# strukturag/libheif

Measured on NVIDIA H100. Metric: megapixels/sec HEIC-grid decode->RGB, higher is better.
Workload: dtype u8

## Files before the change

### libheif_b200/csrc/b200_hevc_entropy.cu

```cuda
#include <cstdint>
#include <cstdlib>
namespace b200 { namespace syn {
__shared__ uint32_t s_kLps4[64];
__shared__ uint8_t s_kTransLps[64];
__shared__ uint8_t s_kNextState[256];
__shared__ unsigned long long s_kState[128];
__shared__ uint8_t s_kInitI[135];
__shared__ uint8_t s_kSigMap4[16];
__shared__ uint8_t s_kScanPos[3][16];
__shared__ uint8_t s_kScanInv[3][16];
__shared__ uint8_t s_kSbInv[4][3][64];
__shared__ uint8_t s_kSigCtx4[3][16];
__shared__ uint8_t s_kSigCtxN[3][4][16];
__shared__ uint8_t s_kChromaTab[4];
__shared__ uint8_t s_kScanX[4][3][64];
__shared__ uint8_t s_kScanY[4][3][64];
} }
#ifdef __CUDA_ARCH__
#define B200_T(name) s_##name
#endif
#include "b200_hevc.h"
static_assert(b200::syn::CTX_COUNT == 135, "s_kInitI above is sized for 135 context variables");

namespace b200 {

#ifndef B200_ENTROPY_WARPS
#define B200_ENTROPY_WARPS 4
#endif
constexpr int EWARPS = B200_ENTROPY_WARPS;

__device__ __forceinline__ unsigned e_ld_acquire(const unsigned* p) {
  unsigned v; asm volatile("ld.relaxed.gpu.global.u32 %0, [%1];" : "=r"(v) : "l"(p) : "memory"); return v;
}
__device__ __forceinline__ void e_st_release(unsigned* p, unsigned v) {
  asm volatile("st.release.gpu.global.u32 [%0], %1;" ::"l"(p), "r"(v) : "memory");
}

struct DevSync {
  unsigned* progress;
  unsigned* sub_done;
  unsigned* error_flag;
  unsigned* queue; unsigned* qtail; unsigned* deps;
  uint32_t dense_tu, dense_coef, dense_tu_cap, dense_coef_cap;
  uint64_t end_bit_position;
  __device__ static void spin_until(const unsigned* p, unsigned need, unsigned* error_flag) {
    if (e_ld_acquire(p) >= need) return;
    unsigned ns = 200, spins = 0;
    for (;;) {
      __nanosleep(ns); if (ns < 8000) ns <<= 1;
      if (e_ld_acquire(p) >= need) return;
      if ((++spins & 63u) != 0) continue;
      if (e_ld_acquire(error_flag)) return;
      if (spins > (1u << 23)) { atomicExch(error_flag, 3u); return; }
    }
  }
  __device__ void wait_row(int row, int need) { spin_until(progress + row, (unsigned)need, error_flag); }
  __device__ void publish_row(int row, int done) { e_st_release(progress + row, (unsigned)done); }
  __device__ void wait_substream(int idx) { spin_until(sub_done + idx, 1u, error_flag); }
  __device__ void finish_substream(int idx, int err) {
    e_st_release(sub_done + idx, 1u);
    if (err) atomicExch(error_flag, (unsigned)err);
  }
  __device__ void notify(int target) {
    if (target < 0) return;
    __threadfence();
    if (atomicSub(deps + target, 1u) == 1u) { const unsigned s = atomicAdd(qtail, 1u); e_st_release(queue + s, (unsigned)target + 1u); }
  }
};

#ifndef B200_ENTROPY_MIN_BLOCKS
#define B200_ENTROPY_MIN_BLOCKS 1
#endif
#ifndef B200_ENTROPY_MAX_BLOCKS_PER_SM
#define B200_ENTROPY_MAX_BLOCKS_PER_SM 0
#endif
template <class Cfg> constexpr int entropy_min_blocks() { return B200_ENTROPY_MIN_BLOCKS; }
template <> constexpr int entropy_min_blocks<syn::CfgCommon>() { return B200_ENTROPY_MIN_BLOCKS > 5 ? B200_ENTROPY_MIN_BLOCKS : 5; }
template <class Cfg>
__global__ void __launch_bounds__(EWARPS * 32, entropy_min_blocks<Cfg>()) hevc_entropy_kernel(const EntropyBatch b) {
  __shared__ __align__(8) syn::U2 s_ctx[EWARPS][syn::CTX_COUNT];
  __shared__ syn::DecoderT<Cfg> s_dec[EWARPS];
  __shared__ DevSync s_sync[EWARPS];
  for (int i = threadIdx.x; i < 64; i += blockDim.x) { syn::s_kLps4[i] = syn::d_kLps4[i]; syn::s_kTransLps[i] = syn::d_kTransLps[i]; }
  for (int i = threadIdx.x; i < syn::CTX_COUNT; i += blockDim.x) syn::s_kInitI[i] = syn::d_kInitI[i];
  for (int i = threadIdx.x; i < 256; i += blockDim.x) syn::s_kNextState[i] = syn::d_kNextState[i];
  for (int i = threadIdx.x; i < 128; i += blockDim.x) syn::s_kState[i] = syn::d_kState[i];
  for (int i = threadIdx.x; i < 16; i += blockDim.x) syn::s_kSigMap4[i] = syn::d_kSigMap4[i];
  for (int i = threadIdx.x; i < 48; i += blockDim.x) { (&syn::s_kScanPos[0][0])[i] = (&syn::d_kScanPos[0][0])[i]; (&syn::s_kScanInv[0][0])[i] = (&syn::d_kScanInv[0][0])[i]; (&syn::s_kSigCtx4[0][0])[i] = (&syn::d_kSigCtx4[0][0])[i]; }
  for (int i = threadIdx.x; i < 192; i += blockDim.x) (&syn::s_kSigCtxN[0][0][0])[i] = (&syn::d_kSigCtxN[0][0][0])[i];
  for (int i = threadIdx.x; i < 768; i += blockDim.x) (&syn::s_kSbInv[0][0][0])[i] = (&syn::d_kSbInv[0][0][0])[i];
  for (int i = threadIdx.x; i < 4; i += blockDim.x) syn::s_kChromaTab[i] = syn::d_kChromaTab[i];
  for (int i = threadIdx.x; i < 4 * 3 * 64; i += blockDim.x) { (&syn::s_kScanX[0][0][0])[i] = (&syn::d_kScanX[0][0][0])[i]; (&syn::s_kScanY[0][0][0])[i] = (&syn::d_kScanY[0][0][0])[i]; }
  __syncthreads();
  if ((threadIdx.x & 31) != 0) return;
  const int slot_w = threadIdx.x >> 5;
  const syn::CtxPtr ctx = (syn::CtxPtr)__cvta_generic_to_shared(s_ctx[slot_w]);
  for (;;) {
    const unsigned slot = atomicAdd(b.qhead, 1u);
    if (slot >= (unsigned)b.nsubs) break;
    unsigned item = e_ld_acquire(b.queue + slot);
    if (!item) {
      unsigned ns = 500, spins = 0;
      for (;;) {
        __nanosleep(ns); if (ns < 16000) ns <<= 1;
        if ((item = e_ld_acquire(b.queue + slot)) != 0u) break;
        if ((++spins & 31u) != 0) continue;
        if (e_ld_acquire(b.error_flag)) return;
        if (spins > (1u << 22)) { atomicExch(b.error_flag, 3u); return; }
      }
    }
    const syn::Substream& gs = b.subs[item - 1u];
    const EntropyPic& ep = b.pics[gs.pic];
    DevSync& sync = s_sync[slot_w];
    sync.progress = b.progress + ep.progress_base; sync.sub_done = b.sub_done + ep.sub_base; sync.error_flag = b.error_flag;
    sync.queue = b.queue; sync.qtail = b.qtail; sync.deps = b.deps;
    sync.dense_tu = sync.dense_coef = sync.dense_tu_cap = sync.dense_coef_cap = 0; sync.end_bit_position = 0;
    syn::run_substream<Cfg>(s_dec[slot_w], ep.sp, ep.pb, b.subs + ep.sub_base, (int)(item - 1u - ep.sub_base), ctx, sync);
  }
}

__global__ void entropy_stats_kernel(const EntropyBatch b, unsigned long long* out2) {
  const int pi = blockIdx.y;
  const EntropyPic& ep = b.pics[pi];
  const int nctb = ep.sp.wctb * ep.sp.hctb;
  unsigned long long tus = 0, coefs = 0;
  for (int a = blockIdx.x * blockDim.x + threadIdx.x; a < nctb; a += gridDim.x * blockDim.x) {
    const CtuInfo ci = ep.pb.ctus[a];
    tus += ci.tu_count;
    for (unsigned k = 0; k < ci.tu_count; k++) { const TuCmd t = ep.pb.tus[ci.tu_start + k]; coefs += (t.w3 & 0x7ff) + ((t.w3 >> 11) & 0x3ff) + ((t.w3 >> 21) & 0x3ff); }
  }
  atomicAdd(out2, tus); atomicAdd(out2 + 1, coefs);
}

__global__ void entropy_gate_kernel(const unsigned* qhead, unsigned need, const unsigned* error_flag) {
// ... 50 lines not shown
```

### libheif_b200/csrc/b200_hevc_syntax.h

```cpp
#pragma once
#include <cstdint>
#include <cstring>
#include "b200_hevc_types.h"

#if defined(__CUDA_ARCH__) && !defined(B200_SYNTAX_HOST_ONLY)
#define B200_SYN_DEVICE 1
#endif
#if defined(__CUDACC__) && !defined(B200_SYNTAX_HOST_ONLY)
#define B200_HDN __host__ __device__ __noinline__
#define B200_NOUNROLL _Pragma("unroll 1")
#define B200_HD __host__ __device__
#define B200_HDI __host__ __device__ __forceinline__
#define B200_TABLE(type, name, dims, ...) static const type h_##name dims = __VA_ARGS__; static __device__ const type d_##name dims = __VA_ARGS__;
#else
#define B200_HDN
#define B200_NOUNROLL
#define B200_HD
#define B200_HDI inline
#define B200_TABLE(type, name, dims, ...) static const type h_##name dims = __VA_ARGS__;
#endif
#if defined(B200_SYN_DEVICE) && !defined(B200_T)
#define B200_T(name) d_##name
#endif
#ifdef B200_SYN_DEVICE
// ... 23 lines not shown
struct U2 { uint32_t x, y; };
typedef U2* CtxPtr;
typedef const uint8_t* TabPtr;
inline U2 ctx_ld(CtxPtr p) { return *p; }
inline void ctx_st(CtxPtr p, U2 v) { *p = v; }
inline CtxPtr ctx_at(CtxPtr base, int i) { return base + i; }
inline uint32_t tab_ld8(TabPtr p, int i) { return p[i]; }
inline uint32_t tab_ld32(TabPtr p, int i) { uint32_t v; memcpy(&v, p + 4 * (size_t)i, 4); return v; }
inline U2 tab_ld64(TabPtr p, int i) { uint64_t v; memcpy(&v, p + 8 * (size_t)i, 8); return U2{(uint32_t)v, (uint32_t)(v >> 32)}; }
#define B200_TADDR(name) (reinterpret_cast<::b200::syn::TabPtr>(&B200_T(name)))
#endif

enum { CTX_SAO_MERGE = 0, CTX_SAO_TYPE = 1, CTX_SPLIT_CU = 2, CTX_PART_MODE = 5, CTX_PREV_INTRA = 6,
       CTX_CHROMA_PRED = 7, CTX_SPLIT_TR = 8, CTX_CBF_LUMA = 11, CTX_CBF_CHROMA = 13, CTX_QP_DELTA = 18,
       CTX_TSKIP = 20, CTX_LAST_X = 22, CTX_LAST_Y = 40, CTX_CSBF = 58, CTX_SIG = 62, CTX_GT1 = 104,
       CTX_GT2 = 128, CTX_TQ_BYPASS = 134, CTX_COUNT = 135, CTX_STRIDE = 144 };

B200_TABLE(uint8_t, kInitI, [CTX_COUNT], {
  153, 200, 139, 141, 157, 184, 184, 63, 153, 138, 138, 111, 141, 94, 138, 182, 154, 154, 154, 154, 139, 139,
  110, 110, 124, 125, 140, 153, 125, 127, 140, 109, 111, 143, 127, 111, 79, 108, 123, 63,
  110, 110, 124, 125, 140, 153, 125, 127, 140, 109, 111, 143, 127, 111, 79, 108, 123, 63,
  91, 171, 134, 141,
  111, 111, 125, 110, 110, 94, 124, 108, 124, 107, 125, 141, 179, 153, 125, 107, 125, 141, 179, 153, 125,
  107, 125, 141, 179, 153, 125, 140, 139, 182, 182, 152, 136, 152, 136, 153, 136, 139, 111, 136, 139, 111,
  140, 92, 137, 138, 140, 152, 138, 139, 153, 74, 149, 92, 139, 107, 122, 152, 140, 179, 166, 182, 140, 227, 122, 197,
  138, 153, 136, 167, 152, 152,
  154})
B200_TABLE(uint32_t, kLps4, [64], {0xf0d0b080u, 0xe3c5a780u, 0xd8bb9e80u, 0xcdb2967bu, 0xc3a98e74u, 0xb9a0876fu, 0xaf988069u, 0xa6907a64u, 0x9e89745fu, 0x96826e5au, 0x8e7b6855u, 0x87756351u, 0x806f5e4du, 0x7a695949u, 0x74645545u, 0x6e5f5042u, 0x685a4c3eu, 0x6356483bu, 0x5e514538u, 0x594d4135u, 0x55493e33u, 0x50453b30u, 0x4c42382eu, 0x483f352bu, 0x453b3229u, 0x41383027u, 0x3e362d25u, 0x3b332b23u, 0x38302921u, 0x352e2720u, 0x322b251eu, 0x3029231du, 0x2d27211bu, 0x2b251f1au, 0x29231e18u, 0x27211c17u, 0x25201b16u, 0x231e1a15u, 0x211d1814u, 0x1f1b1713u, 0x1e1a1612u, 0x1c191511u, 0x1b171410u, 0x1916130fu, 0x1815120eu, 0x1714110eu, 0x1613100du, 0x15120f0cu, 0x14110e0cu, 0x13100e0bu, 0x120f0d0bu, 0x110f0c0au, 0x100e0c0au, 0x0f0d0b09u, 0x0e0c0b09u, 0x0e0c0a08u, 0x0d0b0908u, 0x0c0b0907u, 0x0c0a0907u, 0x0b0a0807u, 0x0b090806u, 0x0a090706u, 0x09080706u, 0x02020202u})
B200_TABLE(uint8_t, kTransLps, [64], {0,0,1,2,2,4,4,5,6,7,8,9,9,11,11,12,13,13,15,15,16,16,18,18,19,19,21,21,22,22,23,24,
  24,25,26,26,27,27,28,29,29,30,30,30,31,32,32,33,33,33,34,34,35,35,35,36,36,36,37,37,37,38,38,63})
B200_TABLE(uint8_t, kSigMap4, [16], {0, 1, 4, 5, 2, 3, 4, 5, 6, 6, 8, 8, 7, 7, 8, 8})
// ... 7 lines not shown
B200_TABLE(uint8_t, kSigCtx4, [3][16], {{0,2,1,6,3,4,7,6,4,5,7,8,5,8,8,8},{0,1,4,5,2,3,4,5,6,6,8,8,7,7,8,8},{0,2,6,7,1,3,6,7,4,4,8,8,5,5,8,8}})
B200_TABLE(uint8_t, kSigCtxN, [3][4][16], {{{2,1,1,1,1,1,0,0,0,0,0,0,0,0,0,0},{2,1,2,0,1,2,0,0,1,2,0,0,1,0,0,0},{2,2,1,2,1,0,2,1,0,0,1,0,0,0,0,0},{2,2,2,2,2,2,2,2,2,2,2,2,2,2,2,2}},{{2,1,1,0,1,1,0,0,1,0,0,0,0,0,0,0},{2,2,2,2,1,1,1,1,0,0,0,0,0,0,0,0},{2,1,0,0,2,1,0,0,2,1,0,0,2,1,0,0},{2,2,2,2,2,2,2,2,2,2,2,2,2,2,2,2}},{{2,1,1,0,1,1,0,0,1,0,0,0,0,0,0,0},{2,1,0,0,2,1,0,0,2,1,0,0,2,1,0,0},{2,2,2,2,1,1,1,1,0,0,0,0,0,0,0,0},{2,2,2,2,2,2,2,2,2,2,2,2,2,2,2,2}}})

B200_HD inline int clip3(int lo, int hi, int v) { return v < lo ? lo : (v > hi ? hi : v); }
B200_HD inline int imin(int a, int b) { return a < b ? a : b; }
#ifdef B200_SYN_DEVICE
B200_HD inline int hi_bit(uint32_t v) { return 31 - __clz((int)v); }
B200_HD inline int lo_bit(uint32_t v) { return __ffs((int)v) - 1; }
B200_HD inline int pop_count(uint32_t v) { return __popc(v); }
#else
B200_HD inline int hi_bit(uint32_t v) { return 31 - __builtin_clz(v); }
B200_HD inline int lo_bit(uint32_t v) { return __builtin_ctz(v); }
B200_HD inline int pop_count(uint32_t v) { return __builtin_popcount(v); }
#endif

struct SeqParams {
  int32_t W, H, log2ctb, wctb, hctb, w4, w8, h8, chroma, bd;
  int32_t log2_min_cb, log2_min_tb, log2_max_tb, max_th_depth_intra;
  int32_t sao_enabled, transform_skip, cu_qp_delta, qg_log2, sign_hiding, wpp, sao_scale_luma, sao_scale_chroma;
  int32_t dense;
  int32_t tu_slots, coef_slots;
  int32_t pcm, pcm_bd_y, pcm_bd_c, pcm_shift_y, pcm_shift_c, log2_min_pcm, log2_max_pcm, pcm_lf_disabled;
  int32_t tq_bypass;
  int32_t tiles;
};

struct Substream {
  uint32_t pic;
  uint32_t byte_begin, byte_end;
  uint32_t ctb_begin, ctb_end;
// ... 104 lines not shown
#endif
      out = (out << t) | (q & ((1u << t) - 1u)); k -= t;
    }
    return out;
  }
  B200_HD inline int terminate(const CabacStream& st) {
    range -= 2;
    if ((val >> 16) >= range) return 1;
    if (range < 256) { range <<= 1; shift(1, st); }
    return 0;
  }
};

B200_HDN inline void init_contexts(CtxPtr ctx, int slice_qp) {
  const int qp = clip3(0, 51, slice_qp);
  for (int i = 0; i < CTX_COUNT; i++) {
    const int iv = B200_T(kInitI)[i], m = (iv >> 4) * 5 - 45, nn = ((iv & 15) << 3) - 16;
    const int pre = clip3(1, 126, ((m * qp) >> 4) + nn);
    const int mps = pre > 63, st = mps ? pre - 64 : 63 - pre;
    ctx_st(ctx_at(ctx, i), tab_ld64(B200_TADDR(kState), (st << 1) | mps));
  }
}

enum { SYN_OK = 0, SYN_E_BITSTREAM = 1, SYN_E_OVERFLOW = 2 };

struct SaoRaw { int8_t type[3], band[3], eo[3]; int8_t off[3][4]; };

struct CfgRuntime { enum : int { chroma = -1, bd = -1, log2_min_cb = -1, log2_min_tb = -1, log2_max_tb = -1, transform_skip = -1, cu_qp_delta = -1, sign_hiding = -1, sao_enabled = -1, wpp = -1, dense = -1, pcm = -1, tq_bypass = -1, tiles = -1 }; };
struct CfgCommon { enum : int { chroma = 1, bd = 8, log2_min_cb = 3, log2_min_tb = 2, log2_max_tb = 5, transform_skip = 0, cu_qp_delta = 1, sign_hiding = 1, sao_enabled = 1, wpp = 1, dense = 0, pcm = 0, tq_bypass = 0, tiles = 0 }; };
B200_HD inline bool matches_common(const SeqParams& q) {
  return q.chroma == 1 && q.bd == 8 && q.log2_min_cb == 3 && q.log2_min_tb == 2 && q.log2_max_tb == 5 && !q.transform_skip && q.cu_qp_delta == 1 && q.sign_hiding == 1 &&
         q.sao_enabled == 1 && q.wpp == 1 && q.dense == 0 && !q.pcm && !q.tq_bypass && !q.tiles;
}
#define B200_SPC(f) ((int)Cfg::f >= 0 ? (int)Cfg::f : (int)sp->f)
#define B200_SPR(f) ((int)Cfg::f >= 0 ? (int)Cfg::f : (int)sp.f)

// ... 133 lines not shown
      int g1ctx = 1, g2 = 0;
      int ctx_set = (i == 0 || c > 0) ? 0 : 2;
      if (carry == 0) ctx_set++;
      const int last_sig = hi_bit(sig), first_sig = lo_bit(sig);
      { unsigned m = sig; const CtxPtr gbase = ctx_at(cx, CTX_GT1 + ctx_set * 4 + (c ? 16 : 0));
        B200_NOUNROLL for (int ng1 = 0; m && ng1 < 8; ng1++) {
          const int kk = hi_bit(m); m ^= 1u << kk;
          if (cb_.bin(ctx_at(gbase, imin(3, g1ctx)), stream)) { g1 |= 1u << kk; g1ctx = 0; } else if (g1ctx > 0) g1ctx++;
        } }
      carry = g1ctx;
      const int last_g1 = g1 ? hi_bit(g1) : -1;
      const bool hidden = sign_hiding && (last_sig - first_sig > 3);
      if (last_g1 >= 0) g2 = cb_.bin(ctx_at(cx, CTX_GT2 + ctx_set + (c ? 4 : 0)), stream);
      const int nsign = pop_count(sig) - (hidden ? 1 : 0);
      const unsigned signs = cb_.bypass_bits(nsign, stream);
      int nsig = 0, sum = 0, rice = 0, sidx = nsign;
      B200_NOUNROLL for (unsigned m = sig; m; nsig++) {
        const int kk = hi_bit(m); m ^= 1u << kk;
        const int base = 1 + (int)((g1 >> kk) & 1) + (kk == last_g1 ? g2 : 0);
        int a = base;
        if (base == ((nsig < 8) ? ((kk == last_g1) ? 3 : 2) : 1)) {
          int pre = 0; B200_NOUNROLL while (pre < 32 && cb_.bypass(stream)) pre++;
          if (pre > 20) { err = SYN_E_BITSTREAM; cabac = cb_; const int count = (int)(cn - coef_n); coef_n = cn; return count; }
          const int rem = (pre <= 3 ? (pre << rice) : (((1 << (pre - 3)) + 3 - 1) << rice)) + (int)cb_.bypass_bits(pre <= 3 ? rice : pre - 3 + rice, stream);
          a = base + rem;
          if (a > 3 * (1 << rice)) rice = imin(rice + 1, 4);
        }
        int neg = 0;
        if (!hidden || kk != first_sig) { sidx--; neg = (int)((signs >> sidx) & 1); }
        int v = neg ? -a : a;
        if (hidden) { sum += a; if (kk == first_sig && (sum & 1)) v = -v; }
        if (cn >= coef_cap) { err = SYN_E_OVERFLOW; cabac = cb_; const int count = (int)(cn - coef_n); coef_n = cn; return count; }
        const int p = (int)tab_ld8(spos, kk);
        CoefEntry e; e.pos = (uint16_t)((((ys << 2) + (p >> 2)) << log2n) + (xs << 2) + (p & 3)); e.level = (int16_t)clip3(-32768, 32767, v);
        pb.coefs[cn++] = e;
      }
    }
    cabac = cb_;
    const int count = (int)(cn - coef_n);
    coef_n = cn;
    return count;
  }

  B200_HDN void mark_tu(int x0, int y0, int log2n) {
    const SliceInfo& sl = pb.slices[ss->slice_idx];
    const int n8 = log2n > 3 ? 1 << (log2n - 3) : 1, bx = x0 >> 3, by = y0 >> 3;
    uint8_t left = 0, top = 0;
    if (!sl.deblocking_disabled) {
      if ((x0 & 7) == 0 && x0 > 0 && (x0 > ctb_x0 || left_lf)) left = 1;
      if ((y0 & 7) == 0 && y0 > 0 && (y0 > ctb_y0 || up_lf)) top = 2;
    }
    uint8_t* e = pb.edge8 + by * sp->w8 + bx;
    if (left) B200_NOUNROLL for (int y = 0; y < n8; y++) e[y * sp->w8] |= left;
    if (top) B200_NOUNROLL for (int x = 0; x < n8; x++) e[x] |= top;
  }

  B200_HDI void transform_unit(const Cu& cu, int x0, int y0, int log2n, int blk, int cbf_l, int cbf_cb, int cbf_cr, int pcb, int pcr) {
    const int cbf_c = B200_SPC(chroma) ? (log2n > 2 ? (cbf_cb | cbf_cr) : (pcb | pcr)) : 0;
    if ((cbf_l || cbf_c) && B200_SPC(cu_qp_delta) && !is_dqp_coded) {
      int v = 0;
      B200_NOUNROLL while (v < 5 && dbin(CTX_QP_DELTA + (v ? 1 : 0))) v++;
      if (v == 5) { int k = 0; B200_NOUNROLL while (k < 16 && dbypass()) { v += 1 << k; k++; } v += (int)dbits(k); }
      if (v && dbypass()) v = -v;
      { const int half = 3 * (B200_SPC(bd) - 8); if (v < -(26 + half) || v > 25 + half) { err = SYN_E_BITSTREAM; return; } }
      is_dqp_coded = 1; dqp_val = v;
      derive_qpy(cu.x0, cu.y0);
    }
    const int pu = cu.nxn ? ((y0 >= cu.y0 + (1 << (cu.log2cb - 1))) ? 2 : 0) + ((x0 >= cu.x0 + (1 << (cu.log2cb - 1))) ? 1 : 0) : 0;
    const int lmode = cu.lmode[pu];
// ... 172 lines not shown
    uint32_t acc = 0; int have = 0;
    B200_NOUNROLL for (int c = 0; c < (chroma ? 3 : 1); c++) {
      const uint32_t cnt = c ? nc : nl; const int bd = c ? sp->pcm_bd_c : sp->pcm_bd_y, sh = c ? sp->pcm_shift_c : sp->pcm_shift_y;
      B200_NOUNROLL for (uint32_t k = 0; k < cnt; k++) {
        B200_NOUNROLL while (have < bd) { acc = (acc << 8) | rbsp_byte(p++); have += 8; }
        have -= bd;
        const uint32_t v = (acc >> have) & ((1u << bd) - 1u);
        acc &= (1u << have) - 1u;
        CoefEntry e; e.pos = (uint16_t)k; e.level = (int16_t)(v << sh);
        pb.coefs[coef_n++] = e;
      }
    }
    cabac.start(stream, p);
    if (!B200_SPC(cu_qp_delta)) cur_qpy = ss->slice_qp; else derive_qpy(x0, y0);
    const int nofilt = sp->pcm_lf_disabled ? 4 : 0;
    B200_NOUNROLL for (int yy = 0; yy < n; yy += 4) B200_NOUNROLL for (int xx = 0; xx < n; xx += 4) pb.ipm4[((y0 + yy) >> 2) * sp->w4 + ((x0 + xx) >> 2)] = 1;
    mark_tu(x0, y0, log2cb);
    B200_NOUNROLL for (int yy = 0; yy < n; yy += 8) B200_NOUNROLL for (int xx = 0; xx < n; xx += 8) {
      const int i8 = ((y0 + yy) >> 3) * sp->w8 + ((x0 + xx) >> 3);
      pb.cd8[i8] = (uint8_t)depth; pb.qp8[i8] = (int8_t)cur_qpy; pb.edge8[i8] |= (uint8_t)nofilt;
    }
    last_cu_qpy = cur_qpy;
    if (cfmt >= 2) {
      emit_block(0, x0, y0, log2cb, 1, 0, 1, coef0, (int)nl, 1u << 21);
      B200_NOUNROLL for (int c = 1; c <= 2; c++) {
        const uint32_t o = coef0 + nl + (uint32_t)(c - 1) * nc;
        if (cfmt == 3) emit_block(c, x0, y0, log2cb, 1, 0, 1, o, (int)nc, 1u << 21);
        else { emit_block(c, x0, y0, log2cb - 1, 1, 0, 1, o, (int)(nc >> 1), 1u << 21); emit_block(c, x0, y0 + (n >> 1), log2cb - 1, 1, 0, 1, o + (nc >> 1), (int)(nc >> 1), 1u << 21); }
      }
      return;
    }
    TuCmd t;
    t.w0 = (uint32_t)(x0 >> 2) | ((uint32_t)(y0 >> 2) << 12) | ((uint32_t)(log2cb - 2) << 24) | (1u << 26) | ((uint32_t)chroma << 27) | ((uint32_t)chroma << 28) | ((uint32_t)chroma << 29);
    t.w1 = 1u | (1u << 6) | ((uint32_t)(cur_qpy + 64) << 12) | (1u << 21) | ((B200_SPC(tq_bypass) && cu_bypass) ? 1u << 22 : 0u);
    t.w2 = coef0;
    t.w3 = nl | (nc << 11) | (nc << 21);
// ... 3 lines not shown
  B200_HDN void chroma_modes_x(Cu& cu, int np) {
    const int cfmt = B200_SPC(chroma);
    B200_NOUNROLL for (int i = 0; i < (cfmt == 3 ? np : 1); i++) {
      int v = 4; if (dbin(CTX_CHROMA_PRED)) v = (int)dbits(2);
      int m;
      if (v == 4) m = cu.lmode[i]; else { m = B200_T(kChromaTab)[v]; if (m == cu.lmode[i]) m = 34; }
      if (cfmt == 2) {
        const unsigned long long w = m < 10 ? 0x207143082082040ull : (m < 20 ? 0x5955134913cd30aull : (m < 30 ? 0x71b6da6596185d7ull : 0x1f79d75cull));
        m = (int)((w >> (6 * (m % 10))) & 63ull);
      }
      cu.cmodes[i] = m;
    }
    cu.cmode = cu.cmodes[0];
  }

  B200_HDI void coding_unit(int x0, int y0, int log2cb, int depth) {
    Cu cu; cu.x0 = x0; cu.y0 = y0; cu.log2cb = log2cb; cu.nxn = 0; cu.cmode = 0;
    const int n = 1 << log2cb;
    if (B200_SPC(tq_bypass)) {
      cu_bypass = dbin(CTX_TQ_BYPASS);
      if (cu_bypass) B200_NOUNROLL for (int yy = 0; yy < n; yy += 8) B200_NOUNROLL for (int xx = 0; xx < n; xx += 8) pb.edge8[((y0 + yy) >> 3) * sp->w8 + ((x0 + xx) >> 3)] |= 4;
    }
    if (log2cb == B200_SPC(log2_min_cb)) cu.nxn = !dbin(CTX_PART_MODE);
    if (cu.nxn && log2cb == 3 && B200_SPC(log2_min_tb) > 2) { err = SYN_E_BITSTREAM; return; }
    if (B200_SPC(pcm) && !cu.nxn && log2cb >= sp->log2_min_pcm && log2cb <= sp->log2_max_pcm && cabac.terminate(stream)) { pcm_unit(x0, y0, log2cb, depth); return; }
    const int np = cu.nxn ? 4 : 1, pbs = cu.nxn ? n / 2 : n;
    int prev[4], mi[4] = {0, 0, 0, 0}, rem[4] = {0, 0, 0, 0};
    B200_NOUNROLL for (int i = 0; i < np; i++) prev[i] = dbin(CTX_PREV_INTRA);
    B200_NOUNROLL for (int i = 0; i < np; i++) { if (prev[i]) { mi[i] = dbypass(); if (mi[i]) mi[i] += dbypass(); } else rem[i] = (int)dbits(5); }
    B200_NOUNROLL for (int i = 0; i < np; i++) {
      const int px = x0 + (i & 1) * pbs, py = y0 + (i >> 1) * pbs;
      const int m = luma_mode(px, py, prev[i], mi[i], rem[i]);
      cu.lmode[i] = m;
      B200_NOUNROLL for (int yy = 0; yy < pbs; yy += 4) B200_NOUNROLL for (int xx = 0; xx < pbs; xx += 4) pb.ipm4[((py + yy) >> 2) * sp->w4 + ((px + xx) >> 2)] = (uint8_t)m;
    }
    if (B200_SPC(chroma) >= 2) chroma_modes_x(cu, np);
    else if (B200_SPC(chroma)) {
      int v = 4; if (dbin(CTX_CHROMA_PRED)) v = (int)dbits(2);
      if (v == 4) cu.cmode = cu.lmode[0]; else { cu.cmode = B200_T(kChromaTab)[v]; if (cu.cmode == cu.lmode[0]) cu.cmode = 34; }
    }
    B200_NOUNROLL for (int yy = 0; yy < n; yy += 8) B200_NOUNROLL for (int xx = 0; xx < n; xx += 8) pb.cd8[((y0 + yy) >> 3) * sp->w8 + ((x0 + xx) >> 3)] = (uint8_t)depth;
    if (!B200_SPC(cu_qp_delta)) cur_qpy = ss->slice_qp; else derive_qpy(x0, y0);
    if (B200_SPC(chroma) >= 2) transform_tree_x(cu, sp->max_th_depth_intra + cu.nxn); else transform_tree(cu, sp->max_th_depth_intra + cu.nxn);
    B200_NOUNROLL for (int yy = 0; yy < n; yy += 8) B200_NOUNROLL for (int xx = 0; xx < n; xx += 8) pb.qp8[((y0 + yy) >> 3) * sp->w8 + ((x0 + xx) >> 3)] = (int8_t)cur_qpy;
    last_cu_qpy = cur_qpy;
  }

  B200_HD inline int cq_levels() const { return sp->log2ctb - B200_SPC(log2_min_cb); }
  B200_HDI void coding_quadtree() {
    const int log2min = B200_SPC(log2_min_cb);
    B200_NOUNROLL for (int i = 0; i < (1 << (2 * cq_levels())) && !err;) {
      int depth = node_depth((unsigned)i, cq_levels());
      B200_NOUNROLL for (;;) {
        const int log2cb = sp->log2ctb - depth, n = 1 << log2cb;
        const int x0 = ctb_x0 + (zx((unsigned)i) << log2min), y0 = ctb_y0 + (zx((unsigned)i >> 1) << log2min);
        if (x0 >= sp->W || y0 >= sp->H) { i += 1 << (2 * (cq_levels() - depth)); break; }
        int split;
        if (x0 + n <= sp->W && y0 + n <= sp->H && log2cb > log2min) {
          int inc = 0;
// ... 18 lines not shown
    cur_ctb_x = rx; cur_ctb_y = ry;
    ctb_x0 = rx << sp->log2ctb; ctb_y0 = ry << sp->log2ctb;
    left_ok = rx > 0 && pb.ctu_slice[addr - 1] == (uint16_t)ss->slice_idx;
    up_ok = ry > 0 && pb.ctu_slice[addr - sp->wctb] == (uint16_t)ss->slice_idx;
    {
      const SliceInfo& cs = pb.slices[ss->slice_idx];
      left_lf = left_ok; up_lf = up_ok;
      if (rx > 0 && !left_ok) { const SliceInfo& o = pb.slices[pb.ctu_slice[addr - 1]]; left_lf = (o.slice_id == cs.slice_id || cs.lf_across_slices) && (o.tile_id == cs.tile_id || cs.lf_across_tiles); }
      if (ry > 0 && !up_ok) { const SliceInfo& o = pb.slices[pb.ctu_slice[addr - sp->wctb]]; up_lf = (o.slice_id == cs.slice_id || cs.lf_across_slices) && (o.tile_id == cs.tile_id || cs.lf_across_tiles); } }
    CtuInfo& ci = pb.ctus[addr];
    ci.slice_idx = (uint16_t)ss->slice_idx;
    if (!B200_SPC(dense)) { tu_n = (uint32_t)addr * (uint32_t)sp->tu_slots; tu_cap = tu_n + (uint32_t)sp->tu_slots; coef_n = (uint32_t)addr * (uint32_t)sp->coef_slots; coef_cap = coef_n + (uint32_t)sp->coef_slots; }
    ctb_tu0 = tu_n;
    if (B200_SPC(sao_enabled)) parse_sao(rx, ry, ci);
    else for (int c = 0; c < 3; c++) { ci.sao[c].type = 0; ci.sao[c].band_or_class = 0; B200_NOUNROLL for (int k = 0; k < 4; k++) ci.sao[c].offset[k] = 0; }
    { const int b0x = rx << (sp->log2ctb - 3), b0y = ry << (sp->log2ctb - 3), nb = 1 << (sp->log2ctb - 3);
      B200_NOUNROLL for (int y = 0; y < nb && b0y + y < sp->h8; y++) B200_NOUNROLL for (int x = 0; x < nb && b0x + x < sp->w8; x++) pb.edge8[(b0y + y) * sp->w8 + b0x + x] = 0; }
    coding_quadtree();
    CtuInfo& ce = pb.ctus[cur_ctb_y * sp->wctb + cur_ctb_x];
    ce.tu_start = ctb_tu0; ce.tu_count = (uint16_t)(tu_n - ctb_tu0);
  }
};

typedef DecoderT<CfgRuntime> Decoder;

template <class Cfg, class Sync>
B200_HD int run_substream(DecoderT<Cfg>& d, const SeqParams& sp, const PicBuffers& pb, const Substream* all, int index, CtxPtr ctx, Sync& sync) {
  const Substream& ss = all[index];
  d.sp = &sp; d.pb = pb; d.ss = &ss; d.ctx = ctx; d.err = SYN_OK;
  d.is_dqp_coded = 0; d.dqp_val = 0; d.qpy_prev_qg = ss.slice_qp; d.last_cu_qpy = ss.slice_qp; d.first_qg = 1; d.cur_qpy = ss.slice_qp; d.cu_bypass = 0;
  d.tu_n = 0; d.coef_n = 0; d.tu_cap = 0; d.coef_cap = 0;
  if (B200_SPR(dense)) {
    d.tu_n = sync.dense_tu; d.coef_n = sync.dense_coef; d.tu_cap = sync.dense_tu_cap; d.coef_cap = sync.dense_coef_cap;
  }
  const int rx0 = (int)(ss.ctb_begin % (uint32_t)sp.wctb), ry0 = (int)(ss.ctb_begin / (uint32_t)sp.wctb);
  if (ss.prev >= 0) {
    sync.wait_substream(ss.prev);
    const uint8_t* st = pb.end_state + (size_t)ss.prev * CTX_STRIDE;
    B200_NOUNROLL for (int i = 0; i < CTX_COUNT; i++) ctx_st(ctx_at(ctx, i), tab_ld64(B200_TADDR(kState), (int)B200_LD_SHARED(st + i) & 127));
    d.last_cu_qpy = (int)(int8_t)B200_LD_SHARED(st + CTX_COUNT); d.first_qg = 0;
  }
  if (ss.init_contexts) init_contexts(ctx, ss.slice_qp);
  if (B200_SPR(wpp) && rx0 == 0 && (!ss.init_contexts || ss.prev >= 0) && ss.ctb_begin != ss.slice_addr_rs) {
    const int xn = 1 << sp.log2ctb, yn = (ry0 - 1) << sp.log2ctb;
    bool tr = ry0 > 0 && xn < sp.W && pb.ctu_slice[(ry0 - 1) * sp.wctb + 1] == (uint16_t)ss.slice_idx;
    (void)yn;
    if (tr) { sync.wait_row(ry0 - 1, 2); const uint8_t* st = pb.wpp_ctx + (size_t)(ry0 - 1) * CTX_STRIDE; B200_NOUNROLL for (int i = 0; i < CTX_COUNT; i++) ctx_st(ctx_at(ctx, i), tab_ld64(B200_TADDR(kState), (int)B200_LD_SHARED(st + i) & 127)); }
    else if (ss.prev < 0) init_contexts(ctx, ss.slice_qp);
    d.first_qg = 1;
  }
  d.stream.d = pb.rbsp; d.stream.size = pb.rbsp_size;
  d.cabac.start(d.stream, ss.byte_begin);
  const bool tiles = B200_SPR(tiles) != 0;
  int rx = rx0, ry = ry0;
  B200_NOUNROLL for (uint32_t left = ss.ctb_end - ss.ctb_begin; left > 0; left--, rx++) {
    if (rx == (int)d.ss->tile_x1) { rx = (int)d.ss->tile_x0; ry++; }
    const uint32_t a = (uint32_t)ry * (uint32_t)d.sp->wctb + (uint32_t)rx;
    if (ry > 0 && !tiles) sync.wait_row(ry - 1, rx + 1);
    if (B200_SPR(wpp) && rx == 0 && a != d.ss->ctb_begin) {
      d.first_qg = 1;
    }
    d.decode_ctb((int)a);
    if (d.err) break;
    rx = d.cur_ctb_x; ry = d.cur_ctb_y;
    if (B200_SPR(wpp) && rx == 1) { uint8_t* st = d.pb.wpp_ctx + (size_t)ry * CTX_STRIDE; B200_NOUNROLL for (int i = 0; i < CTX_COUNT; i++) st[i] = (uint8_t)(ctx_ld(ctx_at(d.ctx, i)).y >> 24); }
    const int end = d.cabac.terminate(d.stream);
    const bool last = left == 1;
    if (end != ((last && d.ss->last_of_segment) ? 1 : 0)) { d.err = SYN_E_BITSTREAM; break; }
    if (last && !d.ss->last_of_segment) { if (!d.cabac.terminate(d.stream)) { d.err = SYN_E_BITSTREAM; break; } }
    if (!tiles) sync.publish_row(ry, rx + 1);
    if (B200_SPR(wpp) && rx == 1) sync.notify(d.ss->wake_ctb2);
    if (d.cabac.pos > d.pb.rbsp_size + 64u) { d.err = SYN_E_BITSTREAM; break; }
  }
  { uint8_t* st = d.pb.end_state + (size_t)index * CTX_STRIDE; B200_NOUNROLL for (int i = 0; i < CTX_COUNT; i++) st[i] = (uint8_t)(ctx_ld(ctx_at(d.ctx, i)).y >> 24); st[CTX_COUNT] = (uint8_t)(int8_t)d.last_cu_qpy; }
  if (B200_SPR(dense)) { sync.dense_tu = d.tu_n; sync.dense_coef = d.coef_n; }
  sync.end_bit_position = d.cabac.bit_position();
  sync.finish_substream(index, d.err);
  if (!d.err) sync.notify(d.ss->wake_end);
  return d.err;
}

}
}
```

Measured before the change: 3945.

## Run HEVC entropy decode with full warps, spreading side-effect loops across lanes

The entropy kernel previously ran one lane per warp. Now all 32 lanes execute the substream decode redundantly, and loops without serial dependencies are split across lanes: context init/load/store, edge/ipm/cd8/qp8 map fills and coefficient emission. Synchronisation points (polling, publish, notify) use a lane-0 shuffle or guard. This aims to cut serial store loops in the CABAC thread, at the cost of running the serial decode redundantly on 32 lanes, adding warp syncs, and risking divergence and convergence bugs. It also adds optional trace instrumentation that is compiled out by default.

```diff
diff --git a/libheif_b200/csrc/b200_hevc_entropy.cu b/libheif_b200/csrc/b200_hevc_entropy.cu
--- a/libheif_b200/csrc/b200_hevc_entropy.cu
+++ b/libheif_b200/csrc/b200_hevc_entropy.cu
@@ -35,6 +35,16 @@
 __device__ __forceinline__ void e_st_release(unsigned* p, unsigned v) {
   asm volatile("st.release.gpu.global.u32 [%0], %1;" ::"l"(p), "r"(v) : "memory");
 }
+__device__ __forceinline__ unsigned e_poll(const unsigned* p) { return __shfl_sync(0xffffffffu, e_ld_acquire(p), 0); }
+__device__ __forceinline__ bool lane0() { return syn::lane_id() == 0; }
+
+#ifdef B200_ENTROPY_TRACE
+constexpr int TRACE_CAP = 1 << 16;
+__device__ unsigned long long g_trace[TRACE_CAP][2];
+__device__ unsigned g_trace_sm[TRACE_CAP];
+__device__ __forceinline__ unsigned long long e_globaltimer() { unsigned long long t; asm volatile("mov.u64 %0, %%globaltimer;" : "=l"(t)); return t; }
+__device__ __forceinline__ unsigned e_smid() { unsigned s; asm volatile("mov.u32 %0, %%smid;" : "=r"(s)); return s; }
+#endif
 
 struct DevSync {
   unsigned* progress;
@@ -44,27 +54,33 @@
   uint32_t dense_tu, dense_coef, dense_tu_cap, dense_coef_cap;
   uint64_t end_bit_position;
   __device__ static void spin_until(const unsigned* p, unsigned need, unsigned* error_flag) {
-    if (e_ld_acquire(p) >= need) return;
+    if (e_poll(p) >= need) return;
     unsigned ns = 200, spins = 0;
     for (;;) {
       __nanosleep(ns); if (ns < 8000) ns <<= 1;
-      if (e_ld_acquire(p) >= need) return;
+      if (e_poll(p) >= need) return;
       if ((++spins & 63u) != 0) continue;
-      if (e_ld_acquire(error_flag)) return;
-      if (spins > (1u << 23)) { atomicExch(error_flag, 3u); return; }
+      if (e_poll(error_flag)) return;
+      if (spins > (1u << 23)) { if (lane0()) atomicExch(error_flag, 3u); return; }
     }
   }
   __device__ void wait_row(int row, int need) { spin_until(progress + row, (unsigned)need, error_flag); }
-  __device__ void publish_row(int row, int done) { e_st_release(progress + row, (unsigned)done); }
+  __device__ void publish_row(int row, int done) { syn::warp_sync(); if (lane0()) e_st_release(progress + row, (unsigned)done); }
   __device__ void wait_substream(int idx) { spin_until(sub_done + idx, 1u, error_flag); }
   __device__ void finish_substream(int idx, int err) {
-    e_st_release(sub_done + idx, 1u);
-    if (err) atomicExch(error_flag, (unsigned)err);
+    syn::warp_sync();
+    if (lane0()) {
+      e_st_release(sub_done + idx, 1u);
+      if (err) atomicExch(error_flag, (unsigned)err);
+    }
   }
   __device__ void notify(int target) {
     if (target < 0) return;
-    __threadfence();
-    if (atomicSub(deps + target, 1u) == 1u) { const unsigned s = atomicAdd(qtail, 1u); e_st_release(queue + s, (unsigned)target + 1u); }
+    syn::warp_sync();
+    if (lane0()) {
+      __threadfence();
+      if (atomicSub(deps + target, 1u) == 1u) { const unsigned s = atomicAdd(qtail, 1u); e_st_release(queue + s, (unsigned)target + 1u); }
+    }
   }
 };
 
@@ -78,7 +94,7 @@
 template <> constexpr int entropy_min_blocks<syn::CfgCommon>() { return B200_ENTROPY_MIN_BLOCKS > 5 ? B200_ENTROPY_MIN_BLOCKS : 5; }
 template <class Cfg>
 __global__ void __launch_bounds__(EWARPS * 32, entropy_min_blocks<Cfg>()) hevc_entropy_kernel(const EntropyBatch b) {
-  __shared__ __align__(8) syn::U2 s_ctx[EWARPS][syn::CTX_COUNT];
+  __shared__ __align__(8) syn::U2 s_ctx[EWARPS][syn::CTX_COUNT + syn::CTX_SCRATCH];
   __shared__ syn::DecoderT<Cfg> s_dec[EWARPS];
   __shared__ DevSync s_sync[EWARPS];
   for (int i = threadIdx.x; i < 64; i += blockDim.x) { syn::s_kLps4[i] = syn::d_kLps4[i]; syn::s_kTransLps[i] = syn::d_kTransLps[i]; }
@@ -92,23 +108,27 @@
   for (int i = threadIdx.x; i < 4; i += blockDim.x) syn::s_kChromaTab[i] = syn::d_kChromaTab[i];
   for (int i = threadIdx.x; i < 4 * 3 * 64; i += blockDim.x) { (&syn::s_kScanX[0][0][0])[i] = (&syn::d_kScanX[0][0][0])[i]; (&syn::s_kScanY[0][0][0])[i] = (&syn::d_kScanY[0][0][0])[i]; }
   __syncthreads();
-  if ((threadIdx.x & 31) != 0) return;
   const int slot_w = threadIdx.x >> 5;
   const syn::CtxPtr ctx = (syn::CtxPtr)__cvta_generic_to_shared(s_ctx[slot_w]);
   for (;;) {
-    const unsigned slot = atomicAdd(b.qhead, 1u);
+    unsigned slot = 0;
+    if (lane0()) slot = atomicAdd(b.qhead, 1u);
+    slot = __shfl_sync(0xffffffffu, slot, 0);
     if (slot >= (unsigned)b.nsubs) break;
-    unsigned item = e_ld_acquire(b.queue + slot);
+    unsigned item = e_poll(b.queue + slot);
     if (!item) {
       unsigned ns = 500, spins = 0;
       for (;;) {
         __nanosleep(ns); if (ns < 16000) ns <<= 1;
-        if ((item = e_ld_acquire(b.queue + slot)) != 0u) break;
+        if ((item = e_poll(b.queue + slot)) != 0u) break;
         if ((++spins & 31u) != 0) continue;
-        if (e_ld_acquire(b.error_flag)) return;
-        if (spins > (1u << 22)) { atomicExch(b.error_flag, 3u); return; }
+        if (e_poll(b.error_flag)) return;
+        if (spins > (1u << 22)) { if (lane0()) atomicExch(b.error_flag, 3u); return; }
       }
     }
+#ifdef B200_ENTROPY_TRACE
+    if (lane0() && item - 1u < (unsigned)TRACE_CAP) { g_trace[item - 1u][0] = e_globaltimer(); g_trace_sm[item - 1u] = e_smid(); }
+#endif
     const syn::Substream& gs = b.subs[item - 1u];
     const EntropyPic& ep = b.pics[gs.pic];
     DevSync& sync = s_sync[slot_w];
@@ -116,8 +136,24 @@
     sync.queue = b.queue; sync.qtail = b.qtail; sync.deps = b.deps;
     sync.dense_tu = sync.dense_coef = sync.dense_tu_cap = sync.dense_coef_cap = 0; sync.end_bit_position = 0;
     syn::run_substream<Cfg>(s_dec[slot_w], ep.sp, ep.pb, b.subs + ep.sub_base, (int)(item - 1u - ep.sub_base), ctx, sync);
-  }
-}
+#ifdef B200_ENTROPY_TRACE
+    if (lane0() && item - 1u < (unsigned)TRACE_CAP) g_trace[item - 1u][1] = e_globaltimer();
+#endif
+  }
+}
+
+#ifdef B200_ENTROPY_TRACE
+extern "C" int b200_debug_entropy_trace(unsigned long long* out, int n) {
+  if (!out || n < 0 || n > TRACE_CAP) return set_error(B200_E_INVALID, "bad trace request");
+  static unsigned long long t[TRACE_CAP][2]; static unsigned sm[TRACE_CAP];
+  cudaError_t e = cudaDeviceSynchronize();
+  if (e == cudaSuccess) e = cudaMemcpyFromSymbol(t, g_trace, sizeof t);
+  if (e == cudaSuccess) e = cudaMemcpyFromSymbol(sm, g_trace_sm, sizeof sm);
+  if (e != cudaSuccess) return set_error(B200_E_CUDA, "entropy trace: %s", cudaGetErrorString(e));
+  for (int i = 0; i < n; i++) { out[3 * i] = t[i][0]; out[3 * i + 1] = t[i][1]; out[3 * i + 2] = sm[i]; }
+  return B200_OK;
+}
+#endif
 
 __global__ void entropy_stats_kernel(const EntropyBatch b, unsigned long long* out2) {
   const int pi = blockIdx.y;
diff --git a/libheif_b200/csrc/b200_hevc_syntax.h b/libheif_b200/csrc/b200_hevc_syntax.h
--- a/libheif_b200/csrc/b200_hevc_syntax.h
+++ b/libheif_b200/csrc/b200_hevc_syntax.h
@@ -1,4 +1,5 @@
 #pragma once
+#include <cassert>
 #include <cstdint>
 #include <cstring>
 #include "b200_hevc_types.h"
@@ -61,7 +62,8 @@
 enum { CTX_SAO_MERGE = 0, CTX_SAO_TYPE = 1, CTX_SPLIT_CU = 2, CTX_PART_MODE = 5, CTX_PREV_INTRA = 6,
        CTX_CHROMA_PRED = 7, CTX_SPLIT_TR = 8, CTX_CBF_LUMA = 11, CTX_CBF_CHROMA = 13, CTX_QP_DELTA = 18,
        CTX_TSKIP = 20, CTX_LAST_X = 22, CTX_LAST_Y = 40, CTX_CSBF = 58, CTX_SIG = 62, CTX_GT1 = 104,
-       CTX_GT2 = 128, CTX_TQ_BYPASS = 134, CTX_COUNT = 135, CTX_STRIDE = 144 };
+       CTX_GT2 = 128, CTX_TQ_BYPASS = 134, CTX_COUNT = 135, CTX_STRIDE = 144,
+       CTX_SCRATCH = 8 };
 
 B200_TABLE(uint8_t, kInitI, [CTX_COUNT], {
   153, 200, 139, 141, 157, 184, 184, 63, 153, 138, 138, 111, 141, 94, 138, 182, 154, 154, 154, 154, 139, 139,
@@ -99,6 +101,24 @@
 B200_HD inline int pop_count(uint32_t v) { return __builtin_popcount(v); }
 #endif
 
+#ifdef __CUDACC__
+__device__ __forceinline__ int lane_id() { unsigned l; asm volatile("mov.u32 %0, %%laneid;" : "=r"(l)); return (int)l; }
+__device__ __forceinline__ void warp_sync() { asm volatile("bar.warp.sync -1;" ::: "memory"); }
+#endif
+#ifdef B200_SYN_DEVICE
+#ifdef B200_ENTROPY_CHECK_CONVERGENCE
+#define B200_LANES_BEGIN() assert(__activemask() == 0xffffffffu)
+#else
+#define B200_LANES_BEGIN() ((void)0)
+#endif
+#define B200_LANE_FOR(k, n) B200_NOUNROLL for (int k = ::b200::syn::lane_id(); k < (n); k += 32)
+#define B200_LANES_END() ::b200::syn::warp_sync()
+#else
+#define B200_LANES_BEGIN() ((void)0)
+#define B200_LANE_FOR(k, n) B200_NOUNROLL for (int k = 0; k < (n); k++)
+#define B200_LANES_END() ((void)0)
+#endif
+
 struct SeqParams {
   int32_t W, H, log2ctb, wctb, hctb, w4, w8, h8, chroma, bd;
   int32_t log2_min_cb, log2_min_tb, log2_max_tb, max_th_depth_intra;
@@ -233,12 +253,25 @@
 
 B200_HDN inline void init_contexts(CtxPtr ctx, int slice_qp) {
   const int qp = clip3(0, 51, slice_qp);
-  for (int i = 0; i < CTX_COUNT; i++) {
+  B200_LANES_BEGIN();
+  B200_LANE_FOR(i, CTX_COUNT) {
     const int iv = B200_T(kInitI)[i], m = (iv >> 4) * 5 - 45, nn = ((iv & 15) << 3) - 16;
     const int pre = clip3(1, 126, ((m * qp) >> 4) + nn);
     const int mps = pre > 63, st = mps ? pre - 64 : 63 - pre;
     ctx_st(ctx_at(ctx, i), tab_ld64(B200_TADDR(kState), (st << 1) | mps));
   }
+  B200_LANES_END();
+}
+
+B200_HDN inline void load_contexts(CtxPtr ctx, const uint8_t* st) {
+  B200_LANES_BEGIN();
+  B200_LANE_FOR(i, CTX_COUNT) ctx_st(ctx_at(ctx, i), tab_ld64(B200_TADDR(kState), (int)B200_LD_SHARED(st + i) & 127));
+  B200_LANES_END();
+}
+B200_HDN inline void store_contexts(CtxPtr ctx, uint8_t* st) {
+  B200_LANES_BEGIN();
+  B200_LANE_FOR(i, CTX_COUNT) st[i] = (uint8_t)(ctx_ld(ctx_at(ctx, i)).y >> 24);
+  B200_LANES_END();
 }
 
 enum { SYN_OK = 0, SYN_E_BITSTREAM = 1, SYN_E_OVERFLOW = 2 };
@@ -402,6 +435,37 @@
       if (last_g1 >= 0) g2 = cb_.bin(ctx_at(cx, CTX_GT2 + ctx_set + (c ? 4 : 0)), stream);
       const int nsign = pop_count(sig) - (hidden ? 1 : 0);
       const unsigned signs = cb_.bypass_bits(nsign, stream);
+#ifdef B200_SYN_DEVICE
+      int nsig = 0, sum = 0, rice = 0;
+      const uint32_t lv = ctx_at(cx, CTX_COUNT);
+      B200_NOUNROLL for (unsigned m = sig; m; nsig++) {
+        const int kk = hi_bit(m); m ^= 1u << kk;
+        const int base = 1 + (int)((g1 >> kk) & 1) + (kk == last_g1 ? g2 : 0);
+        int a = base;
+        if (base == ((nsig < 8) ? ((kk == last_g1) ? 3 : 2) : 1)) {
+          int pre = 0; B200_NOUNROLL while (pre < 32 && cb_.bypass(stream)) pre++;
+          if (pre > 20) { err = SYN_E_BITSTREAM; cabac = cb_; const int count = (int)(cn - coef_n); coef_n = cn; return count; }
+          const int rem = (pre <= 3 ? (pre << rice) : (((1 << (pre - 3)) + 3 - 1) << rice)) + (int)cb_.bypass_bits(pre <= 3 ? rice : pre - 3 + rice, stream);
+          a = base + rem;
+          if (a > 3 * (1 << rice)) rice = imin(rice + 1, 4);
+        }
+        sum += a;
+        asm volatile("st.shared.u32 [%0], %1;" ::"r"(lv + 4u * (uint32_t)kk), "r"(a));
+      }
+      if (cn + (uint32_t)nsig > coef_cap) { err = SYN_E_OVERFLOW; cabac = cb_; const int count = (int)(cn - coef_n); coef_n = cn; return count; }
+      B200_LANES_BEGIN();
+      { const int k = lane_id();
+        if (k < 16 && ((sig >> k) & 1u)) {
+          int a; asm volatile("ld.shared.u32 %0, [%1];" : "=r"(a) : "r"(lv + 4u * (uint32_t)k));
+          const int above = pop_count(sig >> k >> 1);
+          const int neg = (hidden && k == first_sig) ? (sum & 1) : (int)((signs >> (nsign - 1 - above)) & 1u);
+          const int p = (int)tab_ld8(spos, k);
+          CoefEntry e; e.pos = (uint16_t)((((ys << 2) + (p >> 2)) << log2n) + (xs << 2) + (p & 3)); e.level = (int16_t)clip3(-32768, 32767, neg ? -a : a);
+          pb.coefs[cn + (uint32_t)above] = e;
+        } }
+      B200_LANES_END();
+      cn += (uint32_t)nsig;
+#else
       int nsig = 0, sum = 0, rice = 0, sidx = nsign;
       B200_NOUNROLL for (unsigned m = sig; m; nsig++) {
         const int kk = hi_bit(m); m ^= 1u << kk;
@@ -423,6 +487,7 @@
         CoefEntry e; e.pos = (uint16_t)((((ys << 2) + (p >> 2)) << log2n) + (xs << 2) + (p & 3)); e.level = (int16_t)clip3(-32768, 32767, v);
         pb.coefs[cn++] = e;
       }
+#endif
     }
     cabac = cb_;
     const int count = (int)(cn - coef_n);
@@ -439,8 +504,14 @@
       if ((y0 & 7) == 0 && y0 > 0 && (y0 > ctb_y0 || up_lf)) top = 2;
     }
     uint8_t* e = pb.edge8 + by * sp->w8 + bx;
-    if (left) B200_NOUNROLL for (int y = 0; y < n8; y++) e[y * sp->w8] |= left;
-    if (top) B200_NOUNROLL for (int x = 0; x < n8; x++) e[x] |= top;
+    if (!(left | top)) return;
+    B200_LANES_BEGIN();
+    B200_LANE_FOR(k, 2 * n8 - 1) {
+      const bool col = k < n8;
+      const uint8_t v = col ? (uint8_t)(left | (k ? 0 : top)) : top;
+      if (v) e[col ? k * sp->w8 : k - n8 + 1] |= v;
+    }
+    B200_LANES_END();
   }
 
   B200_HDI void transform_unit(const Cu& cu, int x0, int y0, int log2n, int blk, int cbf_l, int cbf_cb, int cbf_cr, int pcb, int pcr) {
@@ -643,12 +714,18 @@
     cabac.start(stream, p);
     if (!B200_SPC(cu_qp_delta)) cur_qpy = ss->slice_qp; else derive_qpy(x0, y0);
     const int nofilt = sp->pcm_lf_disabled ? 4 : 0;
-    B200_NOUNROLL for (int yy = 0; yy < n; yy += 4) B200_NOUNROLL for (int xx = 0; xx < n; xx += 4) pb.ipm4[((y0 + yy) >> 2) * sp->w4 + ((x0 + xx) >> 2)] = 1;
+    { const int l4 = log2cb - 2;
+      B200_LANES_BEGIN();
+      B200_LANE_FOR(k, 1 << (2 * l4)) pb.ipm4[((y0 >> 2) + (k >> l4)) * sp->w4 + (x0 >> 2) + (k & ((1 << l4) - 1))] = 1;
+      B200_LANES_END(); }
     mark_tu(x0, y0, log2cb);
-    B200_NOUNROLL for (int yy = 0; yy < n; yy += 8) B200_NOUNROLL for (int xx = 0; xx < n; xx += 8) {
-      const int i8 = ((y0 + yy) >> 3) * sp->w8 + ((x0 + xx) >> 3);
-      pb.cd8[i8] = (uint8_t)depth; pb.qp8[i8] = (int8_t)cur_qpy; pb.edge8[i8] |= (uint8_t)nofilt;
-    }
+    { const int l8 = log2cb - 3;
+      B200_LANES_BEGIN();
+      B200_LANE_FOR(k, 1 << (2 * l8)) {
+        const int i8 = ((y0 >> 3) + (k >> l8)) * sp->w8 + (x0 >> 3) + (k & ((1 << l8) - 1));
+        pb.cd8[i8] = (uint8_t)depth; pb.qp8[i8] = (int8_t)cur_qpy; pb.edge8[i8] |= (uint8_t)nofilt;
+      }
+      B200_LANES_END(); }
     last_cu_qpy = cur_qpy;
     if (cfmt >= 2) {
       emit_block(0, x0, y0, log2cb, 1, 0, 1, coef0, (int)nl, 1u << 21);
@@ -682,12 +759,18 @@
     cu.cmode = cu.cmodes[0];
   }
 
+  B200_HDI static void fill_cells(uint8_t* m, int stride, int l, uint8_t v, bool set) {
+    B200_LANES_BEGIN();
+    B200_LANE_FOR(k, 1 << (2 * l)) { uint8_t* p = m + (k >> l) * stride + (k & ((1 << l) - 1)); *p = set ? v : (uint8_t)(*p | v); }
+    B200_LANES_END();
+  }
+
   B200_HDI void coding_unit(int x0, int y0, int log2cb, int depth) {
     Cu cu; cu.x0 = x0; cu.y0 = y0; cu.log2cb = log2cb; cu.nxn = 0; cu.cmode = 0;
     const int n = 1 << log2cb;
     if (B200_SPC(tq_bypass)) {
       cu_bypass = dbin(CTX_TQ_BYPASS);
-      if (cu_bypass) B200_NOUNROLL for (int yy = 0; yy < n; yy += 8) B200_NOUNROLL for (int xx = 0; xx < n; xx += 8) pb.edge8[((y0 + yy) >> 3) * sp->w8 + ((x0 + xx) >> 3)] |= 4;
+      if (cu_bypass) fill_cells(pb.edge8 + (y0 >> 3) * sp->w8 + (x0 >> 3), sp->w8, log2cb - 3, 4, false);
     }
     if (log2cb == B200_SPC(log2_min_cb)) cu.nxn = !dbin(CTX_PART_MODE);
     if (cu.nxn && log2cb == 3 && B200_SPC(log2_min_tb) > 2) { err = SYN_E_BITSTREAM; return; }
@@ -700,17 +783,17 @@
       const int px = x0 + (i & 1) * pbs, py = y0 + (i >> 1) * pbs;
       const int m = luma_mode(px, py, prev[i], mi[i], rem[i]);
       cu.lmode[i] = m;
-      B200_NOUNROLL for (int yy = 0; yy < pbs; yy += 4) B200_NOUNROLL for (int xx = 0; xx < pbs; xx += 4) pb.ipm4[((py + yy) >> 2) * sp->w4 + ((px + xx) >> 2)] = (uint8_t)m;
+      fill_cells(pb.ipm4 + (py >> 2) * sp->w4 + (px >> 2), sp->w4, log2cb - cu.nxn - 2, (uint8_t)m, true);
     }
     if (B200_SPC(chroma) >= 2) chroma_modes_x(cu, np);
     else if (B200_SPC(chroma)) {
       int v = 4; if (dbin(CTX_CHROMA_PRED)) v = (int)dbits(2);
       if (v == 4) cu.cmode = cu.lmode[0]; else { cu.cmode = B200_T(kChromaTab)[v]; if (cu.cmode == cu.lmode[0]) cu.cmode = 34; }
     }
-    B200_NOUNROLL for (int yy = 0; yy < n; yy += 8) B200_NOUNROLL for (int xx = 0; xx < n; xx += 8) pb.cd8[((y0 + yy) >> 3) * sp->w8 + ((x0 + xx) >> 3)] = (uint8_t)depth;
+    fill_cells(pb.cd8 + (y0 >> 3) * sp->w8 + (x0 >> 3), sp->w8, log2cb - 3, (uint8_t)depth, true);
     if (!B200_SPC(cu_qp_delta)) cur_qpy = ss->slice_qp; else derive_qpy(x0, y0);
     if (B200_SPC(chroma) >= 2) transform_tree_x(cu, sp->max_th_depth_intra + cu.nxn); else transform_tree(cu, sp->max_th_depth_intra + cu.nxn);
-    B200_NOUNROLL for (int yy = 0; yy < n; yy += 8) B200_NOUNROLL for (int xx = 0; xx < n; xx += 8) pb.qp8[((y0 + yy) >> 3) * sp->w8 + ((x0 + xx) >> 3)] = (int8_t)cur_qpy;
+    fill_cells(reinterpret_cast<uint8_t*>(pb.qp8) + (y0 >> 3) * sp->w8 + (x0 >> 3), sp->w8, log2cb - 3, (uint8_t)(int8_t)cur_qpy, true);
     last_cu_qpy = cur_qpy;
   }
 
@@ -759,8 +842,10 @@
     ctb_tu0 = tu_n;
     if (B200_SPC(sao_enabled)) parse_sao(rx, ry, ci);
     else for (int c = 0; c < 3; c++) { ci.sao[c].type = 0; ci.sao[c].band_or_class = 0; B200_NOUNROLL for (int k = 0; k < 4; k++) ci.sao[c].offset[k] = 0; }
-    { const int b0x = rx << (sp->log2ctb - 3), b0y = ry << (sp->log2ctb - 3), nb = 1 << (sp->log2ctb - 3);
-      B200_NOUNROLL for (int y = 0; y < nb && b0y + y < sp->h8; y++) B200_NOUNROLL for (int x = 0; x < nb && b0x + x < sp->w8; x++) pb.edge8[(b0y + y) * sp->w8 + b0x + x] = 0; }
+    { const int l = sp->log2ctb - 3, b0x = rx << l, b0y = ry << l;
+      B200_LANES_BEGIN();
+      B200_LANE_FOR(k, 1 << (2 * l)) { const int y = b0y + (k >> l), x = b0x + (k & ((1 << l) - 1)); if (y < sp->h8 && x < sp->w8) pb.edge8[y * sp->w8 + x] = 0; }
+      B200_LANES_END(); }
     coding_quadtree();
     CtuInfo& ce = pb.ctus[cur_ctb_y * sp->wctb + cur_ctb_x];
     ce.tu_start = ctb_tu0; ce.tu_count = (uint16_t)(tu_n - ctb_tu0);
@@ -782,7 +867,7 @@
   if (ss.prev >= 0) {
     sync.wait_substream(ss.prev);
     const uint8_t* st = pb.end_state + (size_t)ss.prev * CTX_STRIDE;
-    B200_NOUNROLL for (int i = 0; i < CTX_COUNT; i++) ctx_st(ctx_at(ctx, i), tab_ld64(B200_TADDR(kState), (int)B200_LD_SHARED(st + i) & 127));
+    load_contexts(ctx, st);
     d.last_cu_qpy = (int)(int8_t)B200_LD_SHARED(st + CTX_COUNT); d.first_qg = 0;
   }
   if (ss.init_contexts) init_contexts(ctx, ss.slice_qp);
@@ -790,7 +875,7 @@
     const int xn = 1 << sp.log2ctb, yn = (ry0 - 1) << sp.log2ctb;
     bool tr = ry0 > 0 && xn < sp.W && pb.ctu_slice[(ry0 - 1) * sp.wctb + 1] == (uint16_t)ss.slice_idx;
     (void)yn;
-    if (tr) { sync.wait_row(ry0 - 1, 2); const uint8_t* st = pb.wpp_ctx + (size_t)(ry0 - 1) * CTX_STRIDE; B200_NOUNROLL for (int i = 0; i < CTX_COUNT; i++) ctx_st(ctx_at(ctx, i), tab_ld64(B200_TADDR(kState), (int)B200_LD_SHARED(st + i) & 127)); }
+    if (tr) { sync.wait_row(ry0 - 1, 2); load_contexts(ctx, pb.wpp_ctx + (size_t)(ry0 - 1) * CTX_STRIDE); }
     else if (ss.prev < 0) init_contexts(ctx, ss.slice_qp);
     d.first_qg = 1;
   }
@@ -808,7 +893,7 @@
     d.decode_ctb((int)a);
     if (d.err) break;
     rx = d.cur_ctb_x; ry = d.cur_ctb_y;
-    if (B200_SPR(wpp) && rx == 1) { uint8_t* st = d.pb.wpp_ctx + (size_t)ry * CTX_STRIDE; B200_NOUNROLL for (int i = 0; i < CTX_COUNT; i++) st[i] = (uint8_t)(ctx_ld(ctx_at(d.ctx, i)).y >> 24); }
+    if (B200_SPR(wpp) && rx == 1) store_contexts(d.ctx, d.pb.wpp_ctx + (size_t)ry * CTX_STRIDE);
     const int end = d.cabac.terminate(d.stream);
     const bool last = left == 1;
     if (end != ((last && d.ss->last_of_segment) ? 1 : 0)) { d.err = SYN_E_BITSTREAM; break; }
@@ -817,7 +902,7 @@
     if (B200_SPR(wpp) && rx == 1) sync.notify(d.ss->wake_ctb2);
     if (d.cabac.pos > d.pb.rbsp_size + 64u) { d.err = SYN_E_BITSTREAM; break; }
   }
-  { uint8_t* st = d.pb.end_state + (size_t)index * CTX_STRIDE; B200_NOUNROLL for (int i = 0; i < CTX_COUNT; i++) st[i] = (uint8_t)(ctx_ld(ctx_at(d.ctx, i)).y >> 24); st[CTX_COUNT] = (uint8_t)(int8_t)d.last_cu_qpy; }
+  { uint8_t* st = d.pb.end_state + (size_t)index * CTX_STRIDE; store_contexts(d.ctx, st); st[CTX_COUNT] = (uint8_t)(int8_t)d.last_cu_qpy; }
   if (B200_SPR(dense)) { sync.dense_tu = d.tu_n; sync.dense_coef = d.coef_n; }
   sync.end_bit_position = d.cabac.bit_position();
   sync.finish_substream(index, d.err);
```

Result: faster. 4081, median of 6 (+3.5%).
